# a1q123456/image_stitching

Hardware: AMD Instinct MI355X
Metric: 4K frames stitched/sec (higher is better)
Workload: dtype u8

## Files before the change

image_stitching_amd/csrc/orb.hip:

```cpp
#include "common.h"
#include "dev_math.h"
#include <algorithm>
#include <cmath>
#include <mutex>
#include <unordered_map>

#define ORB_MAX_LEVELS 16
#define ORB_BORDER 32

namespace {

struct LevelDesc {
    int w, h;
    int pp;
    int sp;
    size_t pad_off;
    size_t map_off;
    float scale;
    int nfeat;
    int n2;
    int tiles_x, tiles_y, tile_off;
    int cap1, cand_off;
    int cap2, fin_off;
    int tab_off;
};

struct Levels {
    int n;
    int fast_t, patch, half_patch, edge;
    LevelDesc d[ORB_MAX_LEVELS];
};

struct Work {
    uint8_t *pad, *blur, *score, *nms;
    int* hist;
    int* thr;
    int* tile_cnt;
    uint32_t* surv_xy;
    uint8_t* surv_sc;
    int* cnt1;
    int* cnt2;
    int* flags;
    uint32_t* cand_xy;
    float* cand_resp;
    uint32_t* fin_xy;
    float* fin_resp;
    int* tab;
    int* umax;
    int8_t* pattern;
};

constexpr int ORB_BATCH = 16;
struct OrbIO {
    const uint8_t* src[ORB_BATCH];
    size_t sstride[ORB_BATCH];
    int aligned[ORB_BATCH];
    MisKeyPoint* kps[ORB_BATCH];
    uint32_t* lxy[ORB_BATCH];
    int* n_dev[ORB_BATCH];
    uint8_t* desc[ORB_BATCH];
};
#define WS_OFF(p, f, ws) p = (decltype(p))((const char*)(p) + (size_t)(f) * (ws))

constexpr int GRAY_ROWS = 4;
__global__ __launch_bounds__(256) void gray_kernel(OrbIO io, int w, int h, uint8_t* dst, int pp, size_t ws) {
    const int x = (blockIdx.x * 256 + threadIdx.x) * 4, y0 = blockIdx.y * GRAY_ROWS, f = blockIdx.z;
    if (x >= w) return;
    const uint8_t* bgr = io.src[f];
    const size_t stride = io.sstride[f];
    const int aligned = io.aligned[f];
    WS_OFF(dst, f, ws);
    const int nrows = min(GRAY_ROWS, h - y0);
    if (aligned && x + 4 <= w) {
        unsigned w0[GRAY_ROWS], w1[GRAY_ROWS], w2[GRAY_ROWS];
#pragma unroll
        for (int r = 0; r < GRAY_ROWS; r++) {
            const unsigned* sp = reinterpret_cast<const unsigned*>(bgr + (size_t)min(y0 + r, h - 1) * stride + 3 * (size_t)x);
            w0[r] = sp[0]; w1[r] = sp[1]; w2[r] = sp[2];
        }
#pragma unroll
        for (int r = 0; r < GRAY_ROWS; r++) {
            if (r >= nrows) break;
            const unsigned g0 = ((w0[r] & 255) * 3735 + ((w0[r] >> 8) & 255) * 19235 + ((w0[r] >> 16) & 255) * 9798 + (1 << 14)) >> 15;
            const unsigned g1 = ((w0[r] >> 24) * 3735 + (w1[r] & 255) * 19235 + ((w1[r] >> 8) & 255) * 9798 + (1 << 14)) >> 15;
            const unsigned g2 = (((w1[r] >> 16) & 255) * 3735 + (w1[r] >> 24) * 19235 + (w2[r] & 255) * 9798 + (1 << 14)) >> 15;
            const unsigned g3 = (((w2[r] >> 8) & 255) * 3735 + ((w2[r] >> 16) & 255) * 19235 + (w2[r] >> 24) * 9798 + (1 << 14)) >> 15;
            *reinterpret_cast<unsigned*>(dst + (size_t)(y0 + r + ORB_BORDER) * pp + ORB_BORDER + x) = g0 | (g1 << 8) | (g2 << 16) | (g3 << 24);
        }
    } else {
        for (int r = 0; r < nrows; r++) {
            const uint8_t* s = bgr + (size_t)(y0 + r) * stride + 3 * (size_t)x;
            uint8_t* o = dst + (size_t)(y0 + r + ORB_BORDER) * pp + ORB_BORDER + x;
            for (int k = 0; k < 4 && x + k < w; k++) o[k] = (uint8_t)((s[3 * k] * 3735 + s[3 * k + 1] * 19235 + s[3 * k + 2] * 9798 + (1 << 14)) >> 15);
        }
    }
}

__device__ __forceinline__ unsigned byte_at(unsigned w0, unsigned w1, unsigned w2, int o) {
    const unsigned long long lo = (unsigned long long)w0 | ((unsigned long long)w1 << 32);
    return (o < 8 ? (unsigned)(lo >> (8 * o)) : (w2 >> (8 * (o - 8)))) & 255u;
}
#ifndef MIS_RS_ROWS
#define MIS_RS_ROWS 4
#endif
constexpr int RS_ROWS = MIS_RS_ROWS;
__global__ __launch_bounds__(256) void resize_kernel(const uint8_t* __restrict__ src, int sw, int sh, int spp, uint8_t* __restrict__ dst, int dw, int dh, int dpp,
                                                     const int* __restrict__ tab, size_t ws) {
    const int x = (blockIdx.x * 64 + (threadIdx.x & 63)) * 4;
    const int ybase = __builtin_amdgcn_readfirstlane((blockIdx.y * 4 + (threadIdx.x >> 6)) * RS_ROWS);
    if (x >= dw || ybase >= dh) return;
    WS_OFF(src, blockIdx.z, ws); WS_OFF(dst, blockIdx.z, ws);
    const int dw4 = (dw + 3) & ~3;
    const int *xo = tab, *xm = tab + dw4, *yo = tab + 2 * dw4, *ym = tab + 2 * dw4 + dh;
    const int4 o4 = *reinterpret_cast<const int4*>(xo + x), m4 = *reinterpret_cast<const int4*>(xm + x);
    const int xs[4] = {o4.x, o4.y, o4.z, o4.w}, ms[4] = {m4.x, m4.y, m4.z, m4.w};
    const int nvalid = min(4, dw - x), nrows = min(RS_ROWS, dh - ybase);
    const int base = xs[0] & ~3, last = xs[nvalid - 1] + 1 - base;
    const uint8_t* r0[RS_ROWS];
    const uint8_t* r1[RS_ROWS];
    int my1[RS_ROWS];
#pragma unroll
    for (int r = 0; r < RS_ROWS; r++) {
        const int y = min(ybase + r, dh - 1);
        const int y0 = yo[y], y1 = y0 + 1 < sh ? y0 + 1 : y0;
        my1[r] = ym[y];
        r0[r] = src + (size_t)(y0 + ORB_BORDER) * spp + ORB_BORDER;
        r1[r] = src + (size_t)(y1 + ORB_BORDER) * spp + ORB_BORDER;
    }
    uint8_t* out = dst + (size_t)(ybase + ORB_BORDER) * dpp + ORB_BORDER + x;
    unsigned res[RS_ROWS];
    if (last <= 11) {
        unsigned a[RS_ROWS][3], b[RS_ROWS][3];
#pragma unroll
        for (int r = 0; r < RS_ROWS; r++) {
            const unsigned* p0 = reinterpret_cast<const unsigned*>(r0[r] + base);
            const unsigned* p1 = reinterpret_cast<const unsigned*>(r1[r] + base);
            a[r][0] = p0[0]; a[r][1] = p0[1]; a[r][2] = p0[2]; b[r][0] = p1[0]; b[r][1] = p1[1]; b[r][2] = p1[2];
        }
#pragma unroll
        for (int r = 0; r < RS_ROWS; r++) res[r] = 0;
#pragma unroll
        for (int k = 0; k < 4; k++) {
            const int o = xs[k] - base, mx1 = ms[k], mx0 = 256 - mx1;
            const bool ok = k < nvalid;
            const int oo = ok ? o : 0;
            const bool p1 = oo >= 4, p2 = oo >= 8;
#pragma unroll
            for (int r = 0; r < RS_ROWS; r++) {
                const unsigned alo = p2 ? a[r][2] : (p1 ? a[r][1] : a[r][0]), ahi = p2 ? 0u : (p1 ? a[r][2] : a[r][1]);
                const unsigned blo = p2 ? b[r][2] : (p1 ? b[r][1] : b[r][0]), bhi = p2 ? 0u : (p1 ? b[r][2] : b[r][1]);
                const unsigned ta = __builtin_amdgcn_alignbyte(ahi, alo, (unsigned)oo & 3u), tb = __builtin_amdgcn_alignbyte(bhi, blo, (unsigned)oo & 3u);
                const unsigned h0 = (ta & 255u) * mx0 + ((ta >> 8) & 255u) * mx1;
                const unsigned h1 = (tb & 255u) * mx0 + ((tb >> 8) & 255u) * mx1;
                res[r] |= ok ? ((h0 * (256 - my1[r]) + h1 * my1[r] + (1u << 15)) >> 16) << (8 * k) : 0u;
            }
        }
    } else {
#pragma unroll
        for (int r = 0; r < RS_ROWS; r++) {
            res[r] = 0;
#pragma unroll
            for (int k = 0; k < 4; k++) {
                if (k >= nvalid) break;
                const int x0 = xs[k], x1 = x0 + 1 < sw ? x0 + 1 : x0, mx1 = ms[k], mx0 = 256 - mx1;
                const unsigned h0 = (unsigned)r0[r][x0] * mx0 + (unsigned)r0[r][x1] * mx1;
                const unsigned h1 = (unsigned)r1[r][x0] * mx0 + (unsigned)r1[r][x1] * mx1;
                res[r] |= ((h0 * (256 - my1[r]) + h1 * my1[r] + (1u << 15)) >> 16) << (8 * k);
            }
        }
    }
#pragma unroll
    for (int r = 0; r < RS_ROWS; r++) {
        if (r >= nrows) break;
        uint8_t* o = out + (size_t)r * dpp;
        if (nvalid == 4) *reinterpret_cast<unsigned*>(o) = res[r];
        else
            for (int k = 0; k < nvalid; k++) o[k] = (uint8_t)(res[r] >> (8 * k));
    }
}

template <bool SIDES>
__global__ __launch_bounds__(256) void border_kernel(Levels L, uint8_t* pad, size_t ws) {
    const int f = blockIdx.z / L.n;
    const LevelDesc& d = L.d[blockIdx.z - f * L.n];
    WS_OFF(pad, f, ws);
    const int B = ORB_BORDER, pw = d.w + 2 * B, ph = d.h + 2 * B;
    uint8_t* p = pad + d.pad_off;
    if (!SIDES) {
        const int px4 = (blockIdx.x * 256 + threadIdx.x) * 4;
        if (px4 >= pw) return;
        const bool inner = px4 >= B && px4 + 3 < B + d.w;
        unsigned v[4];
        size_t drow[4], srow[4];
#pragma unroll
        for (int r = 0; r < 4; r++) {
            const int yy = blockIdx.y * 4 + r, py = yy < B ? yy : ph - 2 * B + yy;
            srow[r] = (size_t)(mis_reflect101(py - B, d.h) + B) * d.pp; drow[r] = (size_t)py * d.pp;
        }
        if (inner) {
#pragma unroll
            for (int r = 0; r < 4; r++) v[r] = *reinterpret_cast<const unsigned*>(p + srow[r] + px4);
#pragma unroll
            for (int r = 0; r < 4; r++) *reinterpret_cast<unsigned*>(p + drow[r] + px4) = v[r];
        } else {
#pragma unroll
            for (int r = 0; r < 4; r++)
                for (int k = 0; k < 4 && px4 + k < pw; k++) p[drow[r] + px4 + k] = p[srow[r] + mis_reflect101(px4 + k - B, d.w) + B];
        }
        return;
    }
    const int t = blockIdx.x * 256 + threadIdx.x, row = t >> 4, g = t & 15;
    if (row >= d.h) return;
    const int px = g < 8 ? 4 * g : pw - B + 4 * (g - 8);
    const size_t ro = (size_t)(row + B) * d.pp;
    unsigned v = 0;
#pragma unroll
    for (int k = 0; k < 4; k++) v |= (unsigned)p[ro + mis_reflect101(px + k - B, d.w) + B] << (8 * k);
    if ((px & 3) == 0) *reinterpret_cast<unsigned*>(p + ro + px) = v;
    else
#pragma unroll
        for (int k = 0; k < 4; k++) p[ro + px + k] = (uint8_t)(v >> (8 * k));
}

__device__ __forceinline__ bool fast_pretest(const uint8_t* p, int pp, int t) {
    const int v = p[0], hi = v + t, lo = v - t;
    const int c0 = p[3 * pp], c4 = p[3], c8 = p[-3 * pp], c12 = p[-3];
    unsigned br = (c0 > hi) | ((c4 > hi) << 2) | ((c8 > hi) << 4) | ((c12 > hi) << 6);
    unsigned dk = (c0 < lo) | ((c4 < lo) << 2) | ((c8 < lo) << 4) | ((c12 < lo) << 6);
    const unsigned adj_b = br & ((br >> 2) | (br << 6)), adj_d = dk & ((dk >> 2) | (dk << 6));
    if (!((adj_b | adj_d) & 0x55)) return false;
    const int c2 = p[2 * pp + 2], c6 = p[-2 * pp + 2], c10 = p[-2 * pp - 2], c14 = p[2 * pp - 2];
    br |= ((c2 > hi) << 1) | ((c6 > hi) << 3) | ((c10 > hi) << 5) | ((c14 > hi) << 7);
    dk |= ((c2 < lo) << 1) | ((c6 < lo) << 3) | ((c10 < lo) << 5) | ((c14 < lo) << 7);
    const unsigned b2 = br | (br << 8), d2 = dk | (dk << 8);
    const unsigned rb = b2 & (b2 >> 1) & (b2 >> 2) & (b2 >> 3), rd = d2 & (d2 >> 1) & (d2 >> 2) & (d2 >> 3);
    return ((rb | rd) & 0xff) != 0;
}
__device__ __forceinline__ int fast_score_full(const uint8_t* p, int pp, int t) {
    const int v = p[0];
    int d[16];
    d[0] = v - p[3 * pp]; d[1] = v - p[3 * pp + 1]; d[2] = v - p[2 * pp + 2]; d[3] = v - p[pp + 3];
    d[4] = v - p[3]; d[5] = v - p[-pp + 3]; d[6] = v - p[-2 * pp + 2]; d[7] = v - p[-3 * pp + 1];
    d[8] = v - p[-3 * pp]; d[9] = v - p[-3 * pp - 1]; d[10] = v - p[-2 * pp - 2]; d[11] = v - p[-pp - 3];
    d[12] = v - p[-3]; d[13] = v - p[pp - 3]; d[14] = v - p[2 * pp - 2]; d[15] = v - p[3 * pp - 1];
    int n3[16], x3[16];
#pragma unroll
    for (int i = 0; i < 16; i++) {
        n3[i] = min(min(d[i], d[(i + 1) & 15]), d[(i + 2) & 15]);
        x3[i] = max(max(d[i], d[(i + 1) & 15]), d[(i + 2) & 15]);
    }
    int A = -512, Bm = 512;
#pragma unroll
    for (int i = 0; i < 16; i++) {
        A = max(A, min(min(n3[i], n3[(i + 3) & 15]), n3[(i + 6) & 15]));
        Bm = min(Bm, max(max(x3[i], x3[(i + 3) & 15]), x3[(i + 6) & 15]));
    }
    const int best = max(A, -Bm);
    return best > t ? best - 1 : 0;
}
__device__ __forceinline__ int fast_score_px(const uint8_t* p, int pp, int t) { return fast_pretest(p, pp, t) ? fast_score_full(p, pp, t) : 0; }

#ifndef MIS_FT_ROWS
#define MIS_FT_ROWS 64
#endif
constexpr int FT_COLS = 64, FT_ROWS = MIS_FT_ROWS, FG_PITCH = 96, FG_COL0 = 15, HIST_COPIES = 8;
constexpr int FT_WR = (FT_ROWS + 2 + 3) / 4;
constexpr int FT_SLOTS = FT_COLS * FT_ROWS / 4;
#ifdef MIS_ORB_STATS
__device__ unsigned long long g_orb_stats[8];
#endif
__global__ __launch_bounds__(256) void fast_nms_kernel(Levels L, const uint8_t* pad, int* hist, int* tile_cnt, uint32_t* surv_xy, uint8_t* surv_sc, size_t ws) {
    __shared__ __attribute__((aligned(16))) uint8_t g[(FT_ROWS + 10) * FG_PITCH];
    __shared__ __attribute__((aligned(16))) uint8_t sc[(FT_ROWS + 2) * (FT_COLS + 4)];
    __shared__ int lh[256];
    __shared__ int lcount;
    __shared__ uint32_t lxy[FT_SLOTS];
    __shared__ uint8_t lsc[FT_SLOTS];
    __shared__ unsigned short queue[(FT_ROWS + 2) * (FT_COLS + 2)];
    __shared__ int qcount;
    const int fz = blockIdx.z / L.n, lz = blockIdx.z - fz * L.n;
    const LevelDesc& d = L.d[lz];
    const int x0 = blockIdx.x * FT_COLS, y0 = blockIdx.y * FT_ROWS, t = threadIdx.x;
    if (x0 >= d.w || y0 >= d.h) return;
    WS_OFF(pad, fz, ws); WS_OFF(hist, fz, ws); WS_OFF(tile_cnt, fz, ws); WS_OFF(surv_xy, fz, ws); WS_OFF(surv_sc, fz, ws);
    lh[t] = 0;
    if (t == 0) { lcount = 0; qcount = 0; }
    {
        const int ph = d.h + 2 * ORB_BORDER;
        const uint8_t* src = pad + d.pad_off;
        const int px0 = x0 - 16 + ORB_BORDER, py0 = y0 - 4 + ORB_BORDER;
        for (int i = t; i < (FT_ROWS + 8) * (FG_PITCH / 16); i += 256) {
            const int r = i / (FG_PITCH / 16), c = i - r * (FG_PITCH / 16);
            const int py = min(py0 + r, ph - 1);
            int px = px0 + 16 * c;
            if (px + 15 >= d.pp) px = d.pp - 16;
            reinterpret_cast<uint4*>(g)[i] = *reinterpret_cast<const uint4*>(src + (size_t)py * d.pp + px);
        }
    }
    __syncthreads();
    const int SP = FT_COLS + 4;
    for (int i = t; i < (FT_ROWS + 2) * SP / 4; i += 256) reinterpret_cast<unsigned*>(sc)[i] = 0u;
    {
        const int wv = __builtin_amdgcn_readfirstlane(t >> 6), lane = t & 63;
        const unsigned ft = (unsigned)L.fast_t;
        const int r0 = FT_WR * wv;
        bool pass[FT_WR + 1];
        unsigned long long ball[FT_WR + 1];
        int total = 0;
        {
            const uint8_t* colp = g + r0 * FG_PITCH + (lane + FG_COL0);
            unsigned col[FT_WR + 6];
#pragma unroll
            for (int j = 0; j < FT_WR + 6; j++) col[j] = colp[j * FG_PITCH];
            const int x = x0 - 1 + lane;
            const bool xin = x >= 3 && x < d.w - 3;
            const uint8_t* rowp = g + (r0 + 3) * FG_PITCH + (lane + FG_COL0 - 3);
#pragma unroll
            for (int k = 0; k < FT_WR; k++) {
                const int r = r0 + k, y = y0 - 1 + r;
                const bool rowok = r < FT_ROWS + 2 && y >= 3 && y < d.h - 3;
                const unsigned v = col[k + 3];
                const unsigned dv = max(__builtin_amdgcn_sad_u8(col[k + 6], v, 0u), __builtin_amdgcn_sad_u8(col[k], v, 0u));
                const unsigned dh = max(__builtin_amdgcn_sad_u8(rowp[k * FG_PITCH + 6], v, 0u), __builtin_amdgcn_sad_u8(rowp[k * FG_PITCH], v, 0u));
                pass[k] = rowok & xin & (min(dv, dh) > ft);
                ball[k] = __ballot(pass[k]);
                total += __popcll(ball[k]);
            }
        }
        {
            const int k = lane >> 1, cc = FT_COLS + (lane & 1), r = r0 + k, y = y0 - 1 + r, x = x0 - 1 + cc;
            bool ps = false;
            if (lane < 2 * FT_WR && r < FT_ROWS + 2) {
                const uint8_t* pp = g + (r + 3) * FG_PITCH + (cc + FG_COL0);
                const unsigned v = pp[0];
                const unsigned dv = max(__builtin_amdgcn_sad_u8(pp[3 * FG_PITCH], v, 0u), __builtin_amdgcn_sad_u8(pp[-3 * FG_PITCH], v, 0u));
                const unsigned dh = max(__builtin_amdgcn_sad_u8(pp[3], v, 0u), __builtin_amdgcn_sad_u8(pp[-3], v, 0u));
                ps = x >= 3 && x < d.w - 3 && y >= 3 && y < d.h - 3 && min(dv, dh) > ft;
            }
            pass[FT_WR] = ps;
            ball[FT_WR] = __ballot(ps);
            total += __popcll(ball[FT_WR]);
        }
        int base = 0;
        if (lane == 0 && total) base = atomicAdd(&qcount, total);
        base = __builtin_amdgcn_readfirstlane(base);
        const unsigned long long below = (1ull << lane) - 1ull;
#pragma unroll
        for (int k = 0; k < FT_WR + 1; k++) {
            if (pass[k]) {
                const int r = k < FT_WR ? r0 + k : r0 + (lane >> 1), c = k < FT_WR ? lane : FT_COLS + (lane & 1);
                queue[base + __popcll(ball[k] & below)] = (unsigned short)(r * (FT_COLS + 2) + c);
            }
            base += __popcll(ball[k]);
        }
    }
    __syncthreads();
    for (int q = t; q < qcount; q += 256) {
        const int i = queue[q], r = i / (FT_COLS + 2), c = i - r * (FT_COLS + 2);
        const int fsv = fast_score_full(g + (r + 3) * FG_PITCH + (c + FG_COL0), FG_PITCH, L.fast_t);
        sc[r * SP + c] = (uint8_t)fsv;
#ifdef MIS_ORB_STATS
        if (fsv) atomicAdd(&g_orb_stats[3], 1ull);
#endif
    }
    __syncthreads();
    {
        const int nq = qcount;
        for (int q0 = 0; q0 < nq; q0 += 256) {
            const int q = q0 + t;
            bool keep = false;
            int x = 0, y = 0, v = 0;
            if (q < nq) {
                const int i = queue[q], r = i / (FT_COLS + 2), c = i - r * (FT_COLS + 2);
                const uint8_t* s_ = sc + r * SP + c;
                v = s_[0];
                x = x0 - 1 + c; y = y0 - 1 + r;
                keep = v && r >= 1 && r <= FT_ROWS && c >= 1 && c <= FT_COLS && x >= L.edge && x < d.w - L.edge && y >= L.edge && y < d.h - L.edge &&
                       v > s_[-1] && v > s_[1] && v > s_[-SP - 1] && v > s_[-SP] && v > s_[-SP + 1] && v > s_[SP - 1] && v > s_[SP] && v > s_[SP + 1];
            }
            const unsigned long long m = __ballot(keep);
            int base = 0;
            if ((t & 63) == 0 && m) base = atomicAdd(&lcount, __popcll(m));
            base = __shfl(base, 0);
            if (keep) {
                const int j = base + __popcll(m & ((1ull << (t & 63)) - 1ull));
                lxy[j] = (uint32_t)x | ((uint32_t)y << 16); lsc[j] = (uint8_t)v;
            }
        }
    }
    __syncthreads();
    const int n = lcount;
    const int tile = d.tile_off + blockIdx.y * d.tiles_x + blockIdx.x;
    if (t == 0) tile_cnt[tile] = n;
    if (n == 0) return;
    for (int j = t; j < n; j += 256) {
        atomicAdd(&lh[lsc[j]], 1);
        surv_xy[(size_t)tile * FT_SLOTS + j] = lxy[j]; surv_sc[(size_t)tile * FT_SLOTS + j] = lsc[j];
    }
    __syncthreads();
    if (lh[t]) atomicAdd(&hist[((lz * HIST_COPIES) + ((blockIdx.x + blockIdx.y) & (HIST_COPIES - 1))) * 256 + t], lh[t]);
}

__global__ __launch_bounds__(256) void fast_cut_kernel(Levels L, const int* hist, int* thr, int* flags, size_t ws) {
    __shared__ int suf[256];
    __shared__ int s_thr;
    const int l = blockIdx.x, t = threadIdx.x;
    WS_OFF(hist, blockIdx.y, ws); WS_OFF(thr, blockIdx.y, ws); WS_OFF(flags, blockIdx.y, ws);
    const LevelDesc& d = L.d[l];
    int hsum = 0;
    for (int c = 0; c < HIST_COPIES; c++) hsum += hist[(l * HIST_COPIES + c) * 256 + t];
    suf[t] = t ? hsum : 0;
    __syncthreads();
    for (int o = 1; o < 256; o <<= 1) {
        int add = t + o < 256 ? suf[t + o] : 0;
        __syncthreads();
        suf[t] += add;
        __syncthreads();
    }
    if (t == 0) s_thr = d.n2 == 0 ? 256 : 1;
    __syncthreads();
    if (d.n2 > 0 && suf[1] > d.n2 && t >= 1 && suf[t] >= d.n2 && (t == 255 || suf[t + 1] < d.n2)) s_thr = t;
    __syncthreads();
    if (t == 0) {
        thr[l] = s_thr;
        if (s_thr < 256 && suf[s_thr] > d.cap1) atomicOr(&flags[0], 1);
    }
}

constexpr int CT_TILES = 16;
__global__ __launch_bounds__(256) void compact_kernel(Levels L, const int* tile_cnt, const uint32_t* surv_xy, const uint8_t* surv_sc, const int* thr,
                                                      int* cnt1, uint32_t* cand_xy, float* cand_resp, size_t ws) {
    __shared__ int s_cnt[CT_TILES], s_off[CT_TILES];
    __shared__ int s_base;
    const int l = blockIdx.y, t = threadIdx.x, lane = t & 63, wave = t >> 6;
    WS_OFF(tile_cnt, blockIdx.z, ws); WS_OFF(surv_xy, blockIdx.z, ws); WS_OFF(surv_sc, blockIdx.z, ws); WS_OFF(thr, blockIdx.z, ws);
    WS_OFF(cnt1, blockIdx.z, ws); WS_OFF(cand_xy, blockIdx.z, ws); WS_OFF(cand_resp, blockIdx.z, ws);
    const LevelDesc& d = L.d[l];
    const int ntiles = d.tiles_x * d.tiles_y, first = blockIdx.x * CT_TILES;
    if (first >= ntiles) return;
    const int th = thr[l];
    for (int k = 0; k < CT_TILES / 4; k++) {
        const int slot = wave * (CT_TILES / 4) + k, til = first + slot;
        int cnt = 0;
        if (til < ntiles) {
            const int tile = d.tile_off + til, n = tile_cnt[tile];
            for (int j0 = 0; j0 < n; j0 += 64) {
                const int j = j0 + lane;
                const int v = j < n ? surv_sc[(size_t)tile * FT_SLOTS + j] : 0;
                cnt += __popcll(__ballot(v >= th && v > 0));
            }
        }
        if (lane == 0) s_cnt[slot] = cnt;
    }
    __syncthreads();
    if (t == 0) {
        int tot = 0;
        for (int k = 0; k < CT_TILES; k++) { s_off[k] = tot; tot += s_cnt[k]; }
        s_base = tot ? atomicAdd(&cnt1[l], tot) : 0;
    }
    __syncthreads();
    for (int k = 0; k < CT_TILES / 4; k++) {
        const int slot = wave * (CT_TILES / 4) + k, til = first + slot;
        if (til >= ntiles || s_cnt[slot] == 0) continue;
        const int tile = d.tile_off + til, n = tile_cnt[tile];
        int run = s_base + s_off[slot];
        for (int j0 = 0; j0 < n; j0 += 64) {
            const int j = j0 + lane;
            const int v = j < n ? surv_sc[(size_t)tile * FT_SLOTS + j] : 0;
            const bool keep = v >= th && v > 0;
            const unsigned long long m = __ballot(keep);
            if (keep) {
                const int i = run + __popcll(m & ((1ull << lane) - 1ull));
                if (i < d.cap1) { cand_xy[d.cand_off + i] = surv_xy[(size_t)tile * FT_SLOTS + j]; cand_resp[d.cand_off + i] = (float)v; }
            }
            run += __popcll(m);
        }
    }
}

__global__ void nms_raster_kernel(LevelDesc d, const int* tile_cnt, const uint32_t* surv_xy, const uint8_t* surv_sc, uint8_t* nms) {
    const int ntiles = d.tiles_x * d.tiles_y;
    for (int tl = blockIdx.x; tl < ntiles; tl += gridDim.x) {
        const int tile = d.tile_off + tl, n = tile_cnt[tile];
        for (int j = threadIdx.x; j < n; j += blockDim.x) {
            uint32_t xy = surv_xy[(size_t)tile * FT_SLOTS + j];
            nms[d.map_off + (size_t)(xy >> 16) * d.sp + (xy & 0xffff)] = surv_sc[(size_t)tile * FT_SLOTS + j];
        }
    }
}

__global__ __launch_bounds__(256) void harris_kernel(Levels L, const uint8_t* pad, const int* cnt1, const uint32_t* cand_xy, float* cand_resp, size_t ws) {
    const LevelDesc& d = L.d[blockIdx.y];
    WS_OFF(pad, blockIdx.z, ws); WS_OFF(cnt1, blockIdx.z, ws); WS_OFF(cand_xy, blockIdx.z, ws); WS_OFF(cand_resp, blockIdx.z, ws);
    int i = blockIdx.x * 256 + threadIdx.x;
    int n = min(cnt1[blockIdx.y], d.cap1);
    if (i >= n) return;
    uint32_t xy = cand_xy[d.cand_off + i];
    int x = xy & 0xffff, y = xy >> 16;
    const int pp = d.pp;
    const uint8_t* q0 = pad + d.pad_off + (size_t)(y + ORB_BORDER - 4) * pp + (x + ORB_BORDER - 4);
    const unsigned sh = (unsigned)((uintptr_t)q0 & 3u);
    const uint8_t* a0 = q0 - sh;
    int px[9][9];
#pragma unroll
    for (int r = 0; r < 9; r++) {
        const unsigned* row = reinterpret_cast<const unsigned*>(a0 + (size_t)r * pp);
        const unsigned d0 = row[0], d1 = row[1], d2 = row[2];
        const unsigned w0 = __builtin_amdgcn_alignbyte(d1, d0, sh), w1 = __builtin_amdgcn_alignbyte(d2, d1, sh), w2 = __builtin_amdgcn_alignbyte(0u, d2, sh);
#pragma unroll
        for (int k = 0; k < 4; k++) { px[r][k] = (int)((w0 >> (8 * k)) & 255u); px[r][4 + k] = (int)((w1 >> (8 * k)) & 255u); }
        px[r][8] = (int)(w2 & 255u);
    }
    int a = 0, b = 0, c = 0;
#pragma unroll
    for (int by = 0; by < 7; by++)
#pragma unroll
        for (int bx = 0; bx < 7; bx++) {
            const int Ix = (px[by + 1][bx + 2] - px[by + 1][bx]) * 2 + (px[by][bx + 2] - px[by][bx]) + (px[by + 2][bx + 2] - px[by + 2][bx]);
            const int Iy = (px[by + 2][bx + 1] - px[by][bx + 1]) * 2 + (px[by + 2][bx] - px[by][bx]) + (px[by + 2][bx + 2] - px[by][bx + 2]);
            a += Ix * Ix; b += Iy * Iy; c += Ix * Iy;
        }
    const float scale = 1.f / ((1 << 2) * 7 * 255.f);
    const float scale_sq_sq = scale * scale * scale * scale;
    float fa = (float)a, fb = (float)b, fc = (float)c;
    float s1 = fa * fb, s2 = fc * fc;
    float s3 = 0.04f * (fa + fb);
    s3 = s3 * (fa + fb);
    cand_resp[d.cand_off + i] = ((s1 - s2) - s3) * scale_sq_sq;
}

__device__ __forceinline__ uint32_t fkey(float f) {
    uint32_t u = __float_as_uint(f);
    return (u & 0x80000000u) ? ~u : (u | 0x80000000u);
}

__global__ __launch_bounds__(1024) void select_rank_kernel(Levels L, const int* cnt1, const uint32_t* cand_xy, const float* cand_resp,
                                                            int* cnt2, uint32_t* fin_xy, float* fin_resp, int* flags, int use_harris, size_t ws) {
    WS_OFF(cnt1, blockIdx.y, ws); WS_OFF(cand_xy, blockIdx.y, ws); WS_OFF(cand_resp, blockIdx.y, ws); WS_OFF(cnt2, blockIdx.y, ws);
    WS_OFF(fin_xy, blockIdx.y, ws); WS_OFF(fin_resp, blockIdx.y, ws); WS_OFF(flags, blockIdx.y, ws);
    __shared__ int hist[256];
    __shared__ uint32_t s_prefix, s_mask;
    __shared__ int s_k, s_m;
    __shared__ uint32_t kkey[4096], kxy[4096];
    const int l = blockIdx.x, t = threadIdx.x;
    const LevelDesc& d = L.d[l];
    const int n = min(cnt1[l], d.cap1);
    const uint32_t* xy = cand_xy + d.cand_off;
    const float* rs = cand_resp + d.cand_off;
    const int N = d.nfeat;
    if (N == 0) { if (t == 0) cnt2[l] = 0; return; }
    if (n <= 4096) {
        int P = 1;
        while (P < n) P <<= 1;
        for (int i = t; i < P; i += 1024) {
            if (i < n) { kkey[i] = fkey(rs[i]); kxy[i] = xy[i]; }
            else { kkey[i] = 0; kxy[i] = 0xffffffffu; }
        }
        __syncthreads();
        for (int k = 2; k <= P; k <<= 1)
            for (int j = k >> 1; j > 0; j >>= 1) {
                for (int i = t; i < P; i += 1024) {
                    const int ixj = i ^ j;
                    if (ixj > i) {
                        const uint32_t ka = kkey[i], kb = kkey[ixj], pa = kxy[i], pb = kxy[ixj];
                        const bool a_first = ka > kb || (ka == kb && pa < pb);
                        const bool descending_block = (i & k) == 0;
                        if (a_first != descending_block) { kkey[i] = kb; kkey[ixj] = ka; kxy[i] = pb; kxy[ixj] = pa; }
                    }
                }
                __syncthreads();
            }
        const uint32_t cutk = (use_harris && n > N) ? kkey[N - 1] : 0u;
        if (t == 0) s_m = 0;
        __syncthreads();
        for (int i = t; i < n; i += 1024)
            if (kkey[i] >= cutk && (i == n - 1 || kkey[i + 1] < cutk)) s_m = i + 1;
        __syncthreads();
        const int m = s_m;
// ... 320 lines not shown
    MisContext* ctx = nullptr;
    void (*enqueued_cb)(void*) = nullptr;
    void* enqueued_user = nullptr;
    MisOrbParams p;
    int max_w = 0, max_h = 0;
    int cur_w = 0, cur_h = 0;
    Levels L;
    Work w;
    size_t ws_stride = 0;
    int ws_frames = 0;
    int umax_host[64] = {0};
    int8_t pattern_host[1024] = {0};
    void* mem = nullptr;
    size_t pad_bytes = 0, map_bytes = 0;
    int cand_total = 0, fin_total = 0, tab_total = 0, surv_total = 0, out_cap = 0;
    std::vector<int> tab_host;
    int* host_counts = nullptr;
    bool direct_describe = false;
};

namespace {

void linear_exact_coeffs(int dlen, int slen, int* ofs, int* m1) {
    double inv = (double)dlen / (double)slen, scale = 1.0 / inv;
    for (int i = 0; i < dlen; i++) {
        double v = ((double)i + 0.5) * scale - 0.5;
        int iv = (int)floor(v);
        if (iv < 0) { ofs[i] = 0; m1[i] = 0; }
        else if (iv >= slen - 1) { ofs[i] = slen - 1; m1[i] = 0; }
        else { ofs[i] = iv; m1[i] = (int)lrint((v - (double)iv) * 256.0); }
    }
}

constexpr int ORB_MAX_LEVEL_FEATURES = 2048 - 128;

inline float level_scale(const MisOrbParams& p, int l) { return (float)pow((double)p.scale_factor, (double)l); }
inline int level_dim(int len, float sc) { return (int)lrint((double)((float)len / sc)); }

void level_budgets(const MisOrbParams& p, int* nfeat) {
    float factor = (float)(1.0 / (double)p.scale_factor);
    float nd = (float)p.nfeatures * (1 - factor) / (1 - (float)pow((double)factor, (double)p.nlevels));
    int sum = 0;
    for (int l = 0; l < p.nlevels - 1; l++) { nfeat[l] = (int)lrintf(nd); sum += nfeat[l]; nd *= factor; }
    nfeat[p.nlevels - 1] = std::max(p.nfeatures - sum, 0);
}

int check_level_sizes(MisContext* ctx, const MisOrbParams& p, int w, int h) {
    for (int l = 0; l < p.nlevels; l++) {
        const float sc = level_scale(p, l);
        MIS_CHECK(ctx, level_dim(w, sc) >= 1 && level_dim(h, sc) >= 1, MIS_E_UNSUPPORTED,
                  "ORB level %d of a %dx%d frame is empty (scale_factor %g, nlevels %d)", l, w, h, (double)p.scale_factor, p.nlevels);
    }
    return MIS_OK;
}

void plan_levels(MisOrb* o, int w, int h) {
    Levels& L = o->L;
    const MisOrbParams& p = o->p;
    L.n = p.nlevels; L.fast_t = p.fast_threshold; L.patch = p.patch_size; L.half_patch = p.patch_size / 2; L.edge = p.edge_threshold;
    size_t pad_off = 0, map_off = 0;
    int cand_off = 0, fin_off = 0, tab_off = 0, surv_off = 0;
    int nfeat[ORB_MAX_LEVELS];
    level_budgets(p, nfeat);
    for (int l = 0; l < L.n; l++) {
        LevelDesc& d = L.d[l];
        float sc = level_scale(p, l);
        d.scale = sc;
        d.w = level_dim(w, sc);
        d.h = level_dim(h, sc);
        d.pp = (int)mis_align_up((size_t)d.w + 2 * ORB_BORDER, 64);
        d.sp = (int)mis_align_up((size_t)d.w, 64);
        d.pad_off = pad_off; pad_off += (size_t)d.pp * (d.h + 2 * ORB_BORDER);
        d.map_off = map_off; map_off += (size_t)d.sp * d.h;
        d.nfeat = nfeat[l];
        d.n2 = p.score_type == 0 ? 2 * d.nfeat : d.nfeat;
        d.tiles_x = (d.w + FT_COLS - 1) / FT_COLS; d.tiles_y = (d.h + FT_ROWS - 1) / FT_ROWS;
        d.tile_off = surv_off; surv_off += d.tiles_x * d.tiles_y;
        d.cap1 = 4 * d.n2 + 4096;
        d.cap2 = std::min(d.nfeat + 128, 2048);
        d.cand_off = cand_off; cand_off += d.cap1;
        d.fin_off = fin_off; fin_off += d.cap2;
        d.tab_off = tab_off; tab_off += (2 * ((d.w + 3) & ~3) + 2 * d.h + 3) & ~3;
    }
    o->pad_bytes = pad_off; o->map_bytes = map_off; o->cand_total = cand_off; o->fin_total = fin_off; o->tab_total = tab_off; o->surv_total = surv_off;
    o->tab_host.assign(tab_off, 0);
    for (int l = 1; l < L.n; l++) {
        int* t = o->tab_host.data() + L.d[l].tab_off;
        const int dw4 = (L.d[l].w + 3) & ~3;
        linear_exact_coeffs(L.d[l].w, L.d[l - 1].w, t, t + dw4);
        linear_exact_coeffs(L.d[l].h, L.d[l - 1].h, t + 2 * dw4, t + 2 * dw4 + L.d[l].h);
    }
}

int upload_tables(MisOrb* o) {
    MisContext* ctx = o->ctx;
    if (o->tab_total)
        MIS_HIP(ctx, hipMemcpyAsync(o->w.tab, o->tab_host.data(), sizeof(int) * o->tab_total, hipMemcpyHostToDevice, ctx->stream));
    MIS_HIP(ctx, hipStreamSynchronize(ctx->stream));
    return MIS_OK;
}

std::mutex g_feat_mutex;
std::unordered_map<void*, size_t> g_feat_sizes;

int alloc_features(MisContext* ctx, int cap, int desc_cols, int desc_dtype, MisFeatures* f) {
    size_t kb = mis_align_up(sizeof(MisKeyPoint) * (size_t)cap, 256), db = mis_align_up((size_t)cap * desc_cols * mis_dtype_size(desc_dtype), 256);
    size_t lb = mis_align_up(sizeof(uint32_t) * (size_t)cap, 256);
    void* mem = nullptr;
    size_t got = 0;
    int rc = mis_pool_alloc(ctx, kb + db + lb + 256, &mem, &got);
    if (rc != MIS_OK) return rc;
    f->keypoints = (MisKeyPoint*)mem;
    f->descriptors = (uint8_t*)mem + kb;
    f->desc_cols = desc_cols; f->desc_dtype = desc_dtype;
    f->owner_ = mem;
    f->n = 0;
    std::lock_guard<std::mutex> lock(g_feat_mutex);
    g_feat_sizes[mem] = got;
    return MIS_OK;
}

inline uint32_t* feat_lxy(const MisFeatures* f, int cap) {
    size_t kb = mis_align_up(sizeof(MisKeyPoint) * (size_t)cap, 256), db = mis_align_up((size_t)cap * f->desc_cols * mis_dtype_size(f->desc_dtype), 256);
    return (uint32_t*)((uint8_t*)f->owner_ + kb + db);
}
inline int* feat_count(const MisFeatures* f, int cap) {
    size_t kb = mis_align_up(sizeof(MisKeyPoint) * (size_t)cap, 256), db = mis_align_up((size_t)cap * f->desc_cols * mis_dtype_size(f->desc_dtype), 256);
    size_t lb = mis_align_up(sizeof(uint32_t) * (size_t)cap, 256);
    return (int*)((uint8_t*)f->owner_ + kb + db + lb);
}

int enqueue_detect_group(MisOrb* o, const DevImage* img, int w, int h, MisFeatures* out, int ng) {
    MisContext* ctx = o->ctx;
    const Levels& L = o->L;
    const Work& W = o->w;
    hipStream_t st = ctx->stream;
    const LevelDesc& d0 = L.d[0];
    const size_t ws = o->ws_stride;
    const unsigned nf = (unsigned)ng;
    OrbIO io;
    for (int k = 0; k < ORB_BATCH; k++) {
        const int q = k < ng ? k : 0;
        io.src[k] = (const uint8_t*)img[q].data; io.sstride[k] = img[q].stride;
        io.aligned[k] = (img[q].stride % 4 == 0) && ((uintptr_t)img[q].data % 4 == 0);
        io.kps[k] = out[q].keypoints; io.lxy[k] = feat_lxy(&out[q], o->out_cap); io.n_dev[k] = feat_count(&out[q], o->out_cap);
        io.desc[k] = (uint8_t*)out[q].descriptors;
    }
    MIS_HIP(ctx, hipMemset2DAsync(W.hist, ws ? ws : sizeof(int) * (256 * HIST_COPIES * ORB_MAX_LEVELS + 4 * ORB_MAX_LEVELS), 0,
                                  sizeof(int) * (256 * HIST_COPIES * ORB_MAX_LEVELS + 4 * ORB_MAX_LEVELS), nf, st));
    hipLaunchKernelGGL(gray_kernel, dim3((w + 1023) / 1024, (h + GRAY_ROWS - 1) / GRAY_ROWS, nf), dim3(256), 0, st, io, w, h, W.pad + d0.pad_off, d0.pp, ws);
    for (int l = 1; l < L.n; l++) {
        const LevelDesc &s = L.d[l - 1], &d = L.d[l];
        hipLaunchKernelGGL(resize_kernel, dim3((d.w + 255) / 256, (d.h + 4 * RS_ROWS - 1) / (4 * RS_ROWS), nf), dim3(256), 0, st, W.pad + s.pad_off, s.w, s.h, s.pp, W.pad + d.pad_off, d.w,
                           d.h, d.pp, W.tab + d.tab_off, ws);
    }
    const int pw0 = d0.w + 2 * ORB_BORDER, ph0 = d0.h + 2 * ORB_BORDER;
    hipLaunchKernelGGL((border_kernel<true>), dim3((d0.h * 16 + 255) / 256, 1, L.n * nf), dim3(256), 0, st, L, W.pad, ws);
    hipLaunchKernelGGL((border_kernel<false>), dim3((pw0 + 1023) / 1024, 2 * ORB_BORDER / 4, L.n * nf), dim3(256), 0, st, L, W.pad, ws);
    dim3 gmap((d0.w + FT_COLS - 1) / FT_COLS, (d0.h + FT_ROWS - 1) / FT_ROWS, L.n * nf);
    hipLaunchKernelGGL(fast_nms_kernel, gmap, dim3(256), 0, st, L, W.pad, W.hist, W.tile_cnt, W.surv_xy, W.surv_sc, ws);
    hipLaunchKernelGGL(fast_cut_kernel, dim3(L.n, nf), dim3(256), 0, st, L, W.hist, W.thr, W.flags, ws);
    hipLaunchKernelGGL(compact_kernel, dim3((d0.tiles_x * d0.tiles_y + CT_TILES - 1) / CT_TILES, L.n, nf), dim3(256), 0, st, L, W.tile_cnt, W.surv_xy, W.surv_sc, W.thr, W.cnt1,
                       W.cand_xy, W.cand_resp, ws);
    const int use_harris = o->p.score_type == 0;
    if (use_harris)
        hipLaunchKernelGGL(harris_kernel, dim3((L.d[0].cap1 + 255) / 256, L.n, nf), dim3(256), 0, st, L, W.pad, W.cnt1, W.cand_xy, W.cand_resp, ws);
    hipLaunchKernelGGL(select_rank_kernel, dim3(L.n, nf), dim3(1024), 0, st, L, W.cnt1, W.cand_xy, W.cand_resp, W.cnt2, W.fin_xy, W.fin_resp, W.flags,
                       use_harris, ws);
    hipLaunchKernelGGL(assemble_angle_kernel, dim3((o->out_cap + 3) / 4, nf), dim3(256), 0, st, L, W.pad, W.cnt2, W.fin_xy, W.fin_resp, W.umax, io, o->out_cap, ws, o->direct_describe ? 0 : 1);
    if (o->direct_describe) {
        UMax16 um16;
        for (int v = 0; v < 16; v++) um16.v[v] = o->umax_host[v];
        hipLaunchKernelGGL(describe_direct_kernel, dim3((o->out_cap + 3) / 4, nf), dim3(256), 0, st, L, W.pad, io, W.pattern, W.umax, um16, ws);
    } else {
        for (int k = 0; k < ng; k++) {
            hipLaunchKernelGGL(blur_kernel, dim3((pw0 + 63) / 64, (ph0 + 31) / 32, L.n), dim3(256), 0, st, L, W.pad + k * ws, W.blur + k * ws);
            hipLaunchKernelGGL(describe_kernel, dim3((o->out_cap + 7) / 8), dim3(256), 0, st, L, W.blur + k * ws, out[k].keypoints, io.lxy[k], io.n_dev[k], W.pattern,
                               (uint8_t*)out[k].descriptors);
        }
    }
    MIS_HIP(ctx, hipGetLastError());
    return MIS_OK;
}

int check_image(MisOrb* o, const MisImage* bgr) {
    MisContext* ctx = o->ctx;
    MIS_CHECK(ctx, bgr && bgr->data, MIS_E_INVALID, "null image");
    MIS_CHECK(ctx, bgr->dtype == MIS_U8 && bgr->channels == 3, MIS_E_UNSUPPORTED, "ORB input must be 8UC3 (BGR)");
    MIS_CHECK(ctx, bgr->width <= o->max_w && bgr->height <= o->max_h && bgr->width >= 64 && bgr->height >= 64, MIS_E_INVALID,
              "image %dx%d outside the finder's range (64x64 .. %dx%d)", bgr->width, bgr->height, o->max_w, o->max_h);
    return MIS_OK;
}

int replan_if_needed(MisOrb* o, int w, int h) {
    if (w == o->cur_w && h == o->cur_h) return MIS_OK;
    const int rc = check_level_sizes(o->ctx, o->p, w, h);
    if (rc != MIS_OK) return rc;
    MIS_HIP(o->ctx, hipStreamSynchronize(o->ctx->stream));
    plan_levels(o, w, h);
    o->cur_w = w; o->cur_h = h;
    return upload_tables(o);
}

int orb_alloc_workspace(MisOrb* o, int frames) {
    MisContext* ctx = o->ctx;
    size_t off = 0;
    auto carve = [&](size_t bytes) { size_t o_ = off; off += mis_align_up(bytes, 256); return o_; };
    const bool frame_blur = !o->direct_describe;
    size_t o_pad = carve(o->pad_bytes), o_blur = frame_blur ? carve(o->pad_bytes) : 0;
    size_t o_hist = carve(sizeof(int) * (256 * HIST_COPIES * ORB_MAX_LEVELS + 4 * ORB_MAX_LEVELS)), o_flags = carve(256);
    size_t o_sxy = carve(sizeof(uint32_t) * FT_SLOTS * (size_t)o->surv_total), o_ssc = carve(FT_SLOTS * (size_t)o->surv_total), o_tc = carve(sizeof(int) * (size_t)o->surv_total);
    size_t o_cxy = carve(sizeof(uint32_t) * o->cand_total), o_cr = carve(sizeof(float) * o->cand_total);
    size_t o_fxy = carve(sizeof(uint32_t) * o->fin_total), o_fr = carve(sizeof(float) * o->fin_total);
    size_t o_tab = carve(sizeof(int) * (o->tab_total + 4)), o_umax = carve(sizeof(int) * 64), o_pat = carve(1024);
    const size_t tail = mis_align_up(o->map_bytes, 256) + (frame_blur ? 0 : mis_align_up(o->pad_bytes, 256));
    void* mem = nullptr;
    if (hipMalloc(&mem, off * (size_t)frames + tail) != hipSuccess) return mis_set_error(ctx, MIS_E_NOMEM, "hipMalloc of %zu bytes failed", off * (size_t)frames + tail);
    o->mem = mem; o->ws_stride = off; o->ws_frames = frames;
    uint8_t* m = (uint8_t*)o->mem;
    uint8_t* shared = m + off * (size_t)frames;
    Work& W = o->w;
    W.pad = m + o_pad; W.nms = shared; W.blur = frame_blur ? m + o_blur : shared + mis_align_up(o->map_bytes, 256); W.score = nullptr;
    W.hist = (int*)(m + o_hist); W.thr = W.hist + 256 * HIST_COPIES * ORB_MAX_LEVELS; W.cnt1 = W.thr + ORB_MAX_LEVELS; W.cnt2 = W.cnt1 + ORB_MAX_LEVELS;
    W.surv_xy = (uint32_t*)(m + o_sxy); W.surv_sc = m + o_ssc; W.tile_cnt = (int*)(m + o_tc);
    W.flags = (int*)(m + o_flags);
    W.cand_xy = (uint32_t*)(m + o_cxy); W.cand_resp = (float*)(m + o_cr); W.fin_xy = (uint32_t*)(m + o_fxy); W.fin_resp = (float*)(m + o_fr);
    W.tab = (int*)(m + o_tab); W.umax = (int*)(m + o_umax); W.pattern = (int8_t*)(m + o_pat);
    return MIS_OK;
}

int orb_init_workspace(MisOrb* o) {
    MisContext* ctx = o->ctx;
    const Work& W = o->w;
    MIS_HIP(ctx, hipMemcpyAsync(W.umax, o->umax_host, sizeof(o->umax_host), hipMemcpyHostToDevice, ctx->stream));
    MIS_HIP(ctx, hipMemcpyAsync(W.pattern, o->pattern_host, sizeof(o->pattern_host), hipMemcpyHostToDevice, ctx->stream));
    MIS_HIP(ctx, hipMemset2DAsync(W.flags, o->ws_stride, 0, 256, (size_t)o->ws_frames, ctx->stream));
    MIS_HIP(ctx, hipStreamSynchronize(ctx->stream));
    return upload_tables(o);
}

int orb_ensure_frames(MisOrb* o, int frames) {
    frames = std::min(frames, ORB_BATCH);
    if (o->ws_frames >= frames) return MIS_OK;
    MisContext* ctx = o->ctx;
    MIS_HIP(ctx, hipStreamSynchronize(ctx->stream));
    void* old = o->mem;
    const Work oldw = o->w;
    const size_t olds = o->ws_stride;
    const int oldf = o->ws_frames;
// ... 260 lines not shown
```

Baseline: 3380.

## Pack pyramid levels into dense 1D grids and merge border kernels

Replaces the level-0-sized grids, which launched many empty blocks at the smaller pyramid levels, with packed per-level block offsets. Each block finds its level by a search over prefix offsets. The two border kernels (sides and top/bottom) are merged into a single launch. This removes idle block launches in the border, FAST, compact and Harris stages and one kernel launch, at the cost of a small per-block level lookup and a larger Levels struct passed as a kernel argument.

```diff
diff --git a/image_stitching_amd/csrc/orb.hip b/image_stitching_amd/csrc/orb.hip
--- a/image_stitching_amd/csrc/orb.hip
+++ b/image_stitching_amd/csrc/orb.hip
@@ -28,8 +28,19 @@
 struct Levels {
     int n;
     int fast_t, patch, half_patch, edge;
+    int ft_off[ORB_MAX_LEVELS + 1];
+    int ct_off[ORB_MAX_LEVELS + 1];
+    int bd_off[ORB_MAX_LEVELS + 1];
+    int hr_off[ORB_MAX_LEVELS + 1];
     LevelDesc d[ORB_MAX_LEVELS];
 };
+
+__device__ __forceinline__ int level_of(const int* off, int b) {
+    int l = 0;
+#pragma unroll
+    for (int k = 1; k < ORB_MAX_LEVELS; k++) l = off[k] <= b ? k : l;
+    return l;
+}
 
 struct Work {
     uint8_t *pad, *blur, *score, *nms;
@@ -179,22 +190,20 @@
     }
 }
 
+constexpr int BD_ROW_GROUPS = 2 * ORB_BORDER / 4;
 template <bool SIDES>
-__global__ __launch_bounds__(256) void border_kernel(Levels L, uint8_t* pad, size_t ws) {
-    const int f = blockIdx.z / L.n;
-    const LevelDesc& d = L.d[blockIdx.z - f * L.n];
-    WS_OFF(pad, f, ws);
+__device__ __forceinline__ void border_piece(const LevelDesc& d, uint8_t* pad, int bx, int by) {
     const int B = ORB_BORDER, pw = d.w + 2 * B, ph = d.h + 2 * B;
     uint8_t* p = pad + d.pad_off;
     if (!SIDES) {
-        const int px4 = (blockIdx.x * 256 + threadIdx.x) * 4;
+        const int px4 = (bx * 256 + threadIdx.x) * 4;
         if (px4 >= pw) return;
         const bool inner = px4 >= B && px4 + 3 < B + d.w;
         unsigned v[4];
         size_t drow[4], srow[4];
 #pragma unroll
         for (int r = 0; r < 4; r++) {
-            const int yy = blockIdx.y * 4 + r, py = yy < B ? yy : ph - 2 * B + yy;
+            const int yy = by * 4 + r, py = yy < B ? yy : ph - 2 * B + yy;
             srow[r] = (size_t)(mis_reflect101(py - B, d.h) + B) * d.pp; drow[r] = (size_t)py * d.pp;
         }
         if (inner) {
@@ -209,7 +218,7 @@
         }
         return;
     }
-    const int t = blockIdx.x * 256 + threadIdx.x, row = t >> 4, g = t & 15;
+    const int t = bx * 256 + threadIdx.x, row = t >> 4, g = t & 15;
     if (row >= d.h) return;
     const int px = g < 8 ? 4 * g : pw - B + 4 * (g - 8);
     const size_t ro = (size_t)(row + B) * d.pp;
@@ -220,6 +229,14 @@
     else
 #pragma unroll
         for (int k = 0; k < 4; k++) p[ro + px + k] = (uint8_t)(v >> (8 * k));
+}
+__global__ __launch_bounds__(256) void border_kernel(Levels L, uint8_t* pad, size_t ws) {
+    const int l = level_of(L.bd_off, blockIdx.x);
+    const LevelDesc& d = L.d[l];
+    WS_OFF(pad, blockIdx.y, ws);
+    const int b = blockIdx.x - L.bd_off[l], nside = (d.h * 16 + 255) / 256;
+    if (b < nside) border_piece<true>(d, pad, b, 0);
+    else border_piece<false>(d, pad, (b - nside) / BD_ROW_GROUPS, (b - nside) % BD_ROW_GROUPS);
 }
 
 __device__ __forceinline__ bool fast_pretest(const uint8_t* p, int pp, int t) {
@@ -278,10 +295,10 @@
     __shared__ uint8_t lsc[FT_SLOTS];
     __shared__ unsigned short queue[(FT_ROWS + 2) * (FT_COLS + 2)];
     __shared__ int qcount;
-    const int fz = blockIdx.z / L.n, lz = blockIdx.z - fz * L.n;
+    const int fz = blockIdx.y, lz = level_of(L.ft_off, blockIdx.x);
     const LevelDesc& d = L.d[lz];
-    const int x0 = blockIdx.x * FT_COLS, y0 = blockIdx.y * FT_ROWS, t = threadIdx.x;
-    if (x0 >= d.w || y0 >= d.h) return;
+    const int tl = blockIdx.x - d.tile_off, ty = tl / d.tiles_x, tx = tl - ty * d.tiles_x;
+    const int x0 = tx * FT_COLS, y0 = ty * FT_ROWS, t = threadIdx.x;
     WS_OFF(pad, fz, ws); WS_OFF(hist, fz, ws); WS_OFF(tile_cnt, fz, ws); WS_OFF(surv_xy, fz, ws); WS_OFF(surv_sc, fz, ws);
     lh[t] = 0;
     if (t == 0) { lcount = 0; qcount = 0; }
@@ -390,7 +407,7 @@
     }
     __syncthreads();
     const int n = lcount;
-    const int tile = d.tile_off + blockIdx.y * d.tiles_x + blockIdx.x;
+    const int tile = d.tile_off + ty * d.tiles_x + tx;
     if (t == 0) tile_cnt[tile] = n;
     if (n == 0) return;
     for (int j = t; j < n; j += 256) {
@@ -398,7 +415,7 @@
         surv_xy[(size_t)tile * FT_SLOTS + j] = lxy[j]; surv_sc[(size_t)tile * FT_SLOTS + j] = lsc[j];
     }
     __syncthreads();
-    if (lh[t]) atomicAdd(&hist[((lz * HIST_COPIES) + ((blockIdx.x + blockIdx.y) & (HIST_COPIES - 1))) * 256 + t], lh[t]);
+    if (lh[t]) atomicAdd(&hist[((lz * HIST_COPIES) + ((tx + ty) & (HIST_COPIES - 1))) * 256 + t], lh[t]);
 }
 
 __global__ __launch_bounds__(256) void fast_cut_kernel(Levels L, const int* hist, int* thr, int* flags, size_t ws) {
@@ -432,12 +449,11 @@
                                                       int* cnt1, uint32_t* cand_xy, float* cand_resp, size_t ws) {
     __shared__ int s_cnt[CT_TILES], s_off[CT_TILES];
     __shared__ int s_base;
-    const int l = blockIdx.y, t = threadIdx.x, lane = t & 63, wave = t >> 6;
-    WS_OFF(tile_cnt, blockIdx.z, ws); WS_OFF(surv_xy, blockIdx.z, ws); WS_OFF(surv_sc, blockIdx.z, ws); WS_OFF(thr, blockIdx.z, ws);
-    WS_OFF(cnt1, blockIdx.z, ws); WS_OFF(cand_xy, blockIdx.z, ws); WS_OFF(cand_resp, blockIdx.z, ws);
+    const int l = level_of(L.ct_off, blockIdx.x), t = threadIdx.x, lane = t & 63, wave = t >> 6;
+    WS_OFF(tile_cnt, blockIdx.y, ws); WS_OFF(surv_xy, blockIdx.y, ws); WS_OFF(surv_sc, blockIdx.y, ws); WS_OFF(thr, blockIdx.y, ws);
+    WS_OFF(cnt1, blockIdx.y, ws); WS_OFF(cand_xy, blockIdx.y, ws); WS_OFF(cand_resp, blockIdx.y, ws);
     const LevelDesc& d = L.d[l];
-    const int ntiles = d.tiles_x * d.tiles_y, first = blockIdx.x * CT_TILES;
-    if (first >= ntiles) return;
+    const int ntiles = d.tiles_x * d.tiles_y, first = (blockIdx.x - L.ct_off[l]) * CT_TILES;
     const int th = thr[l];
     for (int k = 0; k < CT_TILES / 4; k++) {
         const int slot = wave * (CT_TILES / 4) + k, til = first + slot;
@@ -490,10 +506,11 @@
 }
 
 __global__ __launch_bounds__(256) void harris_kernel(Levels L, const uint8_t* pad, const int* cnt1, const uint32_t* cand_xy, float* cand_resp, size_t ws) {
-    const LevelDesc& d = L.d[blockIdx.y];
-    WS_OFF(pad, blockIdx.z, ws); WS_OFF(cnt1, blockIdx.z, ws); WS_OFF(cand_xy, blockIdx.z, ws); WS_OFF(cand_resp, blockIdx.z, ws);
-    int i = blockIdx.x * 256 + threadIdx.x;
-    int n = min(cnt1[blockIdx.y], d.cap1);
+    const int l = level_of(L.hr_off, blockIdx.x);
+    const LevelDesc& d = L.d[l];
+    WS_OFF(pad, blockIdx.y, ws); WS_OFF(cnt1, blockIdx.y, ws); WS_OFF(cand_xy, blockIdx.y, ws); WS_OFF(cand_resp, blockIdx.y, ws);
+    int i = (blockIdx.x - L.hr_off[l]) * 256 + threadIdx.x;
+    int n = min(cnt1[l], d.cap1);
     if (i >= n) return;
     uint32_t xy = cand_xy[d.cand_off + i];
     int x = xy & 0xffff, y = xy >> 16;
@@ -980,6 +997,16 @@
         d.fin_off = fin_off; fin_off += d.cap2;
         d.tab_off = tab_off; tab_off += (2 * ((d.w + 3) & ~3) + 2 * d.h + 3) & ~3;
     }
+    int ct = 0, bd = 0, hr = 0;
+    for (int l = 0; l <= ORB_MAX_LEVELS; l++) {
+        L.ft_off[l] = l < L.n ? L.d[l].tile_off : surv_off;
+        L.ct_off[l] = ct; L.bd_off[l] = bd; L.hr_off[l] = hr;
+        if (l >= L.n) continue;
+        const LevelDesc& d = L.d[l];
+        ct += (d.tiles_x * d.tiles_y + CT_TILES - 1) / CT_TILES;
+        bd += (d.h * 16 + 255) / 256 + (d.w + 2 * ORB_BORDER + 1023) / 1024 * BD_ROW_GROUPS;
+        hr += (d.cap1 + 255) / 256;
+    }
     o->pad_bytes = pad_off; o->map_bytes = map_off; o->cand_total = cand_off; o->fin_total = fin_off; o->tab_total = tab_off; o->surv_total = surv_off;
     o->tab_host.assign(tab_off, 0);
     for (int l = 1; l < L.n; l++) {
@@ -1053,16 +1080,14 @@
                            d.h, d.pp, W.tab + d.tab_off, ws);
     }
     const int pw0 = d0.w + 2 * ORB_BORDER, ph0 = d0.h + 2 * ORB_BORDER;
-    hipLaunchKernelGGL((border_kernel<true>), dim3((d0.h * 16 + 255) / 256, 1, L.n * nf), dim3(256), 0, st, L, W.pad, ws);
-    hipLaunchKernelGGL((border_kernel<false>), dim3((pw0 + 1023) / 1024, 2 * ORB_BORDER / 4, L.n * nf), dim3(256), 0, st, L, W.pad, ws);
-    dim3 gmap((d0.w + FT_COLS - 1) / FT_COLS, (d0.h + FT_ROWS - 1) / FT_ROWS, L.n * nf);
-    hipLaunchKernelGGL(fast_nms_kernel, gmap, dim3(256), 0, st, L, W.pad, W.hist, W.tile_cnt, W.surv_xy, W.surv_sc, ws);
+    hipLaunchKernelGGL(border_kernel, dim3(L.bd_off[L.n], nf), dim3(256), 0, st, L, W.pad, ws);
+    hipLaunchKernelGGL(fast_nms_kernel, dim3(L.ft_off[L.n], nf), dim3(256), 0, st, L, W.pad, W.hist, W.tile_cnt, W.surv_xy, W.surv_sc, ws);
     hipLaunchKernelGGL(fast_cut_kernel, dim3(L.n, nf), dim3(256), 0, st, L, W.hist, W.thr, W.flags, ws);
-    hipLaunchKernelGGL(compact_kernel, dim3((d0.tiles_x * d0.tiles_y + CT_TILES - 1) / CT_TILES, L.n, nf), dim3(256), 0, st, L, W.tile_cnt, W.surv_xy, W.surv_sc, W.thr, W.cnt1,
+    hipLaunchKernelGGL(compact_kernel, dim3(L.ct_off[L.n], nf), dim3(256), 0, st, L, W.tile_cnt, W.surv_xy, W.surv_sc, W.thr, W.cnt1,
                        W.cand_xy, W.cand_resp, ws);
     const int use_harris = o->p.score_type == 0;
     if (use_harris)
-        hipLaunchKernelGGL(harris_kernel, dim3((L.d[0].cap1 + 255) / 256, L.n, nf), dim3(256), 0, st, L, W.pad, W.cnt1, W.cand_xy, W.cand_resp, ws);
+        hipLaunchKernelGGL(harris_kernel, dim3(L.hr_off[L.n], nf), dim3(256), 0, st, L, W.pad, W.cnt1, W.cand_xy, W.cand_resp, ws);
     hipLaunchKernelGGL(select_rank_kernel, dim3(L.n, nf), dim3(1024), 0, st, L, W.cnt1, W.cand_xy, W.cand_resp, W.cnt2, W.fin_xy, W.fin_resp, W.flags,
                        use_harris, ws);
     hipLaunchKernelGGL(assemble_angle_kernel, dim3((o->out_cap + 3) / 4, nf), dim3(256), 0, st, L, W.pad, W.cnt2, W.fin_xy, W.fin_resp, W.umax, io, o->out_cap, ws, o->direct_describe ? 0 : 1);
```

New measurement: 3315, median of 2. -1.9%, worse.
